# dlilien/ImpDAR

Measured on AMD Instinct MI355X. Metric: migrated traces/sec + achieved HBM GB/s, Kirchhoff 10000x4096 radargram, higher is better.
Workload: dtype f32; 1 GPU; Kirchhoff diffraction-sum migration, 10000 traces x 4096 samples, constant velocity 1.69e8 m/s, dx 1 m, dt 10 ns (BASELINE config 3); kernel=fast, pairs_total=189920188078, pairs_rank0=189920188078, parallelism=output-trace blocks x1, exchange of input-image rows: allgather

## Files before the change

### impdar_amd/csrc/kirch_plan.h

```cpp
#pragma once
#include "common.h"
#include "kirch_route.h"
#include <vector>

#define KF_PAD_ROWS 128

struct impdar_kirch_plan : KirchGeometry, KirchRoute {
    impdar_ctx *ctx = nullptr;
    KirchKnobs knobs;
    int dtype = IMPDAR_F32, snum = 0, tnum = 0, nranks = 1;
    int nearfield = 0;
    int grad_uniform = 0;
    double grad_h = 1.0, vel = 0;
    DevBuf d_XK, d_XW, d_XW2, d_xhmax;
    int xntab = 0;
    bool xtab_ready = false;
    int diag_tables_built = 0;
    bool table_built[2] = {false, false};
    DevBuf d_dist, d_tt, d_zs, d_zs2, d_ga, d_gb, d_gc;
    DevBuf GT[2], DT[2];
    int buf = 0;
    bool migrated_since_prep = false;
    const void *last_out = nullptr;
    int last_out_buf = 0;
    hipEvent_t ev_ready[2] = {nullptr, nullptr};
    hipEvent_t ev_free[2] = {nullptr, nullptr};
    bool free_recorded[2] = {false, false};
    DevBuf d_hmax, d_klo, d_khi;
    DevBuf d_TK[2], d_TW[2], d_TW2[2], d_c1, d_c2, d_fin, d_WIN;
    int nrows = 0, mrow0 = 0;
    int nb = 0, ntab = 0;
    std::vector<int> h_hmax;
    DevBuf d_queue;
    int slots = 0;
    DevBuf d_partial;
    DevBuf d_tilemap;
    std::vector<short> h_tilemap;
    int tm_key[5] = {-1, -1, -1, -1, -1};
    DevBuf d_ga32, d_ga2_32, d_alo2, d_jr;
    std::vector<double> h_dist, h_zs2min;
    std::vector<int2> h_jr;
    int jr_key[2] = {-1, -1};
    int ntie_groups = 0;
    DevBuf d_tie_ti, d_tie_off, d_tie_n;
    DevBuf d_c1d, d_c2d, d_find;
    std::vector<int> h_half;
    int nchunks = 0;
    static constexpr int NSLOT = 64;
    hipEvent_t evs[NSLOT][6] = {};
    bool haves[NSLOT][3] = {};
    int slot = 0;

    ~impdar_kirch_plan()
    {
        for (hipEvent_t e : {ev_ready[0], ev_ready[1], ev_free[0], ev_free[1]})
            if (e) (void)hipEventDestroy(e);
        for (int s = 0; s < NSLOT; ++s)
            for (int i = 0; i < 6; ++i)
                if (evs[s][i]) (void)hipEventDestroy(evs[s][i]);
    }
};

static inline char *img_row0(const impdar_kirch_plan *p, const DevBuf &b)
{
    return reinterpret_cast<char *>(b.p) + (size_t)KF_PAD_ROWS * p->snum * impdar_dtype_size(p->dtype);
}

static int upload(DevBuf &b, const void *src, size_t bytes)
{
    IMPDAR_HIP_CHECK(b.ensure(bytes ? bytes : 8));
    if (bytes) IMPDAR_HIP_CHECK(hipMemcpy(b.p, src, bytes, hipMemcpyHostToDevice));
    return IMPDAR_OK;
}

int kirch_launch_gen(impdar_kirch_plan *p, void *d_out, int xlo, int xhi, hipStream_t st);
```

### impdar_amd/csrc/kirch_route.h

```cpp
#pragma once
#include "../../include/impdar_hip.h"
#include <algorithm>
#include <cmath>
#include <cstdlib>
#include <cstring>
#include <vector>

#if defined(__HIPCC__)
#define KIRCH_HD __host__ __device__
#else
#define KIRCH_HD
#endif

#define KF_THREADS 256
#define KF_W 512

#define KQ_GS 1056
KIRCH_HD constexpr int kq_ring_slots(int xb) { return ((xb + 15 + 7) / 8) * 8; }
KIRCH_HD constexpr int kq_piece_bytes(int xb) { return ((kq_ring_slots(xb) / 8 * KQ_GS + 255) / 256) * 256; }
KIRCH_HD constexpr int kq_piece_bytes_lk(int xb, int lk) { return (((kq_ring_slots(xb) / 8 + lk) * KQ_GS + 255) / 256) * 256; }
static_assert(kq_piece_bytes_lk(40, 0) == 7424 && kq_piece_bytes_lk(40, 1) == 8448 && kq_piece_bytes_lk(24, 0) == 5376, "");
static_assert(kq_ring_slots(24) == 40 && kq_piece_bytes(24) == 5376 && kq_ring_slots(32) == 48 && kq_piece_bytes(32) == 6400 &&
              kq_ring_slots(40) == 56 && kq_piece_bytes(40) == 7424, "");
KIRCH_HD constexpr int kd_ring_slots(int xb) { return ((xb + 7 + 3) / 4) * 4; }
// ... 398 lines not shown
    std::vector<double> load(8, 0.0);
    std::vector<std::pair<double, int>> cost(units);
    for (int c = 0; c < nchunks; ++c) {
        const int hm = h_hmax[c];
        for (int u = 0; u < units; ++u) {
            double w = 0;
            for (int t = u * G; t < std::min((u + 1) * G, nxt); ++t) {
                const int x0 = x00 + t * tile_w;
                const int nlo = std::max(-hm, -(x0 + tile_w - 1)), nhi = std::min(hm, tnum - 1 - x0);
                const int blocks = std::max(0, nhi - nlo + step_block) / step_block;
                w += ((blocks + ring_blocks - 1) / ring_blocks) * ring_blocks + 8;
            }
            cost[u] = {w, u};
        }
        std::sort(cost.begin(), cost.end(), [](const std::pair<double, int> &a, const std::pair<double, int> &b) {
            return a.first > b.first || (a.first == b.first && a.second < b.second);
        });
        int used[8] = {0, 0, 0, 0, 0, 0, 0, 0};
        for (const auto &cu : cost) {
            int best = -1;
            for (int x = 0; x < 8; ++x)
                if (used[x] < cap && (best < 0 || load[x] < load[best])) best = x;
            for (int g = 0; g < G; ++g) {
                const int t = cu.second * G + g;
                map[((size_t)c * tiles_per_xcd + (size_t)used[best] * G + g) * 8 + best] = (short)(t < nxt ? t : -1);
            }
            ++used[best];
            load[best] += cu.first;
        }
    }
    return map;
}

#ifdef KIRCH_ROUTE_PROBE
static inline KirchKnobs kirch_probe_knobs(const int *k)
{
    KirchKnobs K;
    K.xb_set = k[0], K.xb = k[1], K.nh_set = k[2], K.nh = k[3], K.lk_set = k[4], K.lk = k[5], K.parts_set = k[6], K.parts = k[7];
    K.nhd_set = k[8], K.nhd = k[9], K.xbd_set = k[10], K.xbd = k[11], K.impl = k[12], K.exact_impl = k[13], K.tiefix_off = k[14];
    return K;
}

extern "C" int impdar_kirch_route_probe(int dtype, int snum, int tnum, const double *dist_m, const double *tt_sec, double vel, int nearfield,
                                        int mode, int nranks, const double *tmax_override, int caller_tables, const int *knobs,
                                        long long tie_count, long long tie_cap, int *ints, double *dbls)
{
    const KirchGeometry G = kirch_geometry(snum, tnum, dist_m, tt_sec, vel, tmax_override);
    KirchRoute R = kirch_route(G, dtype, snum, tnum, nranks, nearfield, mode, kirch_probe_knobs(knobs), caller_tables != 0);
    if (R.status == IMPDAR_OK && tie_count >= 0) kirch_route_after_ties(R, tie_count, tie_cap);
    const int I[23] = {R.status, R.mode, R.status == IMPDAR_OK ? R.kernel() : -1, R.tnum_pad, R.gen, R.genW, R.quad, R.dquad, R.xb, R.nh, R.lk, R.quadW,
                       R.quadSH, R.walk_parts_log2, R.want_tie_scan, R.xtab_off, R.tie_ambiguous, R.want_tie_groups, G.increasing, G.uni_t,
                       G.uni_t11, G.uni_x, G.dist_sorted};
    const double D[10] = {G.tmax, G.dt, G.dx, G.xnoise, G.sa, G.alpha, G.hest, G.gen_need, R.err_limit, R.err_sa};
    std::copy(I, I + 23, ints);
    std::copy(D, D + 10, dbls);
    return 0;
}

extern "C" int impdar_kirch_tables_probe(int dtype, int snum, int tnum, const double *dist_m, const double *tt_sec, double vel, int nearfield,
                                         int mode, int nranks, const int *knobs, int *sizes, int *h_half, float *c32 ,
                                         double *c64 , float *gen2 , double *gen_chunk ,
                                         int *hmax, int *klo, int *khi, int *win)
{
    const KirchGeometry G = kirch_geometry(snum, tnum, dist_m, tt_sec, vel, nullptr);
    const KirchRoute R = kirch_route(G, dtype, snum, tnum, nranks, nearfield, mode, kirch_probe_knobs(knobs), false);
    if (R.status != IMPDAR_OK || !G.increasing) return -1;
// ... 14 lines not shown
        std::copy(T.zs2min.begin(), T.zs2min.end(), gen_chunk + T.alo2.size());
    }
    if (G.uniform && ((R.mode == IMPDAR_KIRCH_FAST && !R.gen) || R.dquad)) {
        const KirchRingTables T = kirch_ring_tables(G, R, tt_sec, snum, tnum, h);
        const int S[8] = {T.nchunks, T.nb, T.ntab, T.nrows, T.mrow0, T.tkbytes >= ((size_t)1 << 31), (int)T.win.size(), 0};
        std::copy(S, S + 8, sizes);
        if (hmax) std::copy(T.hmax.begin(), T.hmax.end(), hmax);
        if (klo) std::copy(T.klo.begin(), T.klo.end(), klo);
        if (khi) std::copy(T.khi.begin(), T.khi.end(), khi);
        if (win) std::copy(T.win.begin(), T.win.end(), win);
    }
    return 0;
}

extern "C" int impdar_kirch_ties_probe(int *ties, int n, int *g_ti, int *g_off, int *g_n)
{
    std::vector<KirchTie> list(n);
    if (n) memcpy(list.data(), ties, (size_t)n * sizeof(KirchTie));
    const KirchTieGroups T = kirch_group_ties(list);
    std::copy(T.g_ti.begin(), T.g_ti.end(), g_ti);
    std::copy(T.g_off.begin(), T.g_off.end(), g_off);
    std::copy(T.g_n.begin(), T.g_n.end(), g_n);
    return (int)T.g_ti.size();
}

extern "C" int impdar_kirch_tilemap_probe(const int *h_hmax, int nchunks, int tnum, int xlo, int xhi, int tile_w, int align_mask, int ring_blocks,
                                          int step_block, int G, int tiles_per_xcd, short *map)
{
    const std::vector<short> m = kirch_tilemap(std::vector<int>(h_hmax, h_hmax + nchunks), tnum, xlo, xhi, tile_w, align_mask, ring_blocks,
                                               step_block, G, tiles_per_xcd, nchunks);
    std::copy(m.begin(), m.end(), map);
    return (int)m.size();
}
#endif
```

### impdar_amd/csrc/kirchhoff.hip

```cpp
#include "common.h"
#include "kirch_plan.h"
#include <limits>
#include <cmath>
#include <algorithm>
#include <chrono>
#include <memory>
#include <thread>


struct PrepParams {
    const void *data;
    int ld;
    int snum, nloc, jlo;
    void *GT;
    void *DT;
    int grad_uniform;
    int precomputed;
    double grad_h;
    const double *ga, *gb, *gc;
    int clean;
    int i8;
};

template <typename TI, typename TO>
// ... 1570 lines not shown
    if (hipSetDevice(ctx->device) != hipSuccess) {
        impdar_set_error("hipSetDevice(%d) failed: %s", ctx->device, hipGetErrorString(hipGetLastError()));
        return IMPDAR_ERR_HIP;
    }
    const bool own = caller && !caller->standard;
    int rc;
    if ((rc = kirch_alloc_images(p.get())) ||
        (rc = kirch_upload_axes(p.get(), dist_m, tt_sec, ga, gb, gc, own ? caller->zs : nullptr, own ? caller->zs2 : nullptr)) ||
        (p->want_tie_scan && (rc = kirch_tie_scan(p.get()))) ||
        (p->gen && (rc = kirch_upload_gen_tables(p.get(), dist_m, tt_sec))) ||
        (((p->mode == IMPDAR_KIRCH_FAST && !p->gen) || p->dquad) && (rc = kirch_upload_ring_tables(p.get(), tt_sec))) ||
        (rc = kirch_create_events(p.get())))
        return rc;
    *out = p.release();
    return IMPDAR_OK;
}

extern "C" int impdar_kirch_plan_create(impdar_ctx *ctx, int dtype, int snum, int tnum,
                                        const double *dist_m, const double *tt_sec, double vel,
                                        int nearfield, int grad_uniform, double grad_h,
                                        const double *ga, const double *gb, const double *gc,
                                        int mode, int nranks, impdar_kirch_plan **out)
{
    return kirch_plan_create_impl(ctx, dtype, snum, tnum, dist_m, tt_sec, vel, nearfield, grad_uniform, grad_h, ga, gb, gc, mode, nranks,
                                  KirchKnobs::from_env(), nullptr, out);
}

extern "C" void impdar_kirch_plan_destroy(impdar_kirch_plan *p)
{
    if (!p) return;
    (void)hipSetDevice(p->ctx->device);
    (void)hipStreamSynchronize(p->ctx->aux);
    (void)hipStreamSynchronize(p->ctx->stream);
    delete p;
}

extern "C" int impdar_kirch_plan_mode(const impdar_kirch_plan *p) { return p ? p->mode : IMPDAR_ERR_ARG; }
extern "C" double impdar_kirch_plan_xnoise(const impdar_kirch_plan *p) { return p ? p->xnoise : -1.0; }
extern "C" int impdar_kirch_plan_tnum_pad(const impdar_kirch_plan *p) { return p ? p->tnum_pad : IMPDAR_ERR_ARG; }
extern "C" int impdar_kirch_plan_kernel(const impdar_kirch_plan *p) { return p ? p->kernel() : IMPDAR_ERR_ARG; }

static int prep_image(impdar_kirch_plan *p, const void *d_data, int ld, int jlo, int nloc, int precomputed, int b, hipStream_t st)
{
    PrepParams P;
    P.data = d_data;
    P.ld = ld;
    P.snum = p->snum;
    P.nloc = nloc;
    P.jlo = jlo;
    P.GT = img_row0(p, p->GT[b]);
    P.DT = p->nearfield ? img_row0(p, p->DT[b]) : nullptr;
    P.grad_uniform = p->grad_uniform;
    P.precomputed = precomputed;
    P.grad_h = p->grad_h;
    P.ga = p->d_ga.as<double>();
    P.gb = p->d_gb.as<double>();
    P.gc = p->d_gc.as<double>();
    P.clean = (p->mode == IMPDAR_KIRCH_FAST) ? 1 : (p->dquad ? 2 : 0);
    P.i8 = (p->quad || p->dquad) ? 1 : 0;
    dim3 grid((nloc + 63) / 64, (p->snum + 63) / 64);
    if (p->dtype == IMPDAR_F32 && P.i8)
        hipLaunchKernelGGL((kirch_prep_direct_kernel<float, 8>), dim3((nloc + 255) / 256, p->snum), dim3(256), 0, st, P);
    else if (p->dquad)
        hipLaunchKernelGGL((kirch_prep_direct_kernel<double, 4>), dim3((nloc + 255) / 256, p->snum), dim3(256), 0, st, P);
    else if (p->dtype == IMPDAR_F32)
        hipLaunchKernelGGL((kirch_prep_kernel<float, float>), grid, dim3(256), 0, st, P);
// ... 63 lines not shown
        p->haves[p->slot][0] = p->haves[p->slot][1] = p->haves[p->slot][2] = false;
    }
    const int b = p->buf;
    if (p->free_recorded[b] && !more) IMPDAR_HIP_CHECK(hipStreamWaitEvent(st, p->ev_free[b], 0));
    if (p->ctx->produced) IMPDAR_HIP_CHECK(hipStreamWaitEvent(st, p->ctx->ev_produced, 0));
    if (p->last_out && d_data == p->last_out && p->free_recorded[p->last_out_buf])
        IMPDAR_HIP_CHECK(hipStreamWaitEvent(st, p->ev_free[p->last_out_buf], 0));
    hipEvent_t *ev = p->evs[p->slot];
    if (!p->haves[p->slot][0]) IMPDAR_HIP_CHECK(hipEventRecord(ev[0], st));
    int rc;
    if (nloc > 0 && (rc = prep_image(p, d_data, ld, jlo, nloc, precomputed, b, st))) return rc;
    if ((p->mode == IMPDAR_KIRCH_FAST && p->quad) || p->dquad)
        rc = prep_table_ring(p, b, st);
    else
        rc = (p->mode == IMPDAR_KIRCH_FAST && !p->gen) ? prep_table_tab(p, b, st) : IMPDAR_OK;
    if (rc) return rc;
    IMPDAR_HIP_CHECK(hipEventRecord(ev[1], st));
    IMPDAR_HIP_CHECK(hipEventRecord(p->ev_ready[b], st));
    p->haves[p->slot][0] = true;
    return IMPDAR_OK;
}

extern "C" int impdar_kirch_prep(impdar_kirch_plan *p, const void *d_data, int ld, int jlo, int nloc)
{
    return kirch_prep_impl(p, d_data, ld, jlo, nloc, 0);
}

int impdar_kirch_prep_precomputed(impdar_kirch_plan *p, const void *d_grad, int ld, int jlo, int nloc)
{
    return kirch_prep_impl(p, d_grad, ld, jlo, nloc, 1);
}

static int build_tilemap(impdar_kirch_plan *p, FastParams &P, int tile_w, int align_mask, int ring_blocks, int step_block,
                         hipStream_t st)
{
    P.tilemap = nullptr;
    const int key[5] = {P.xlo, P.xhi, tile_w, P.G, P.tiles_per_xcd};
    const size_t n = (size_t)P.nchunks * P.tiles_per_xcd * 8;
    if (memcmp(key, p->tm_key, sizeof(key)) != 0 || p->h_tilemap.size() != n) {
        std::vector<short> map = kirch_tilemap(p->h_hmax, p->tnum, P.xlo, P.xhi, tile_w, align_mask, ring_blocks, step_block, P.G,
                                               P.tiles_per_xcd, P.nchunks);
        if (map.empty()) return IMPDAR_OK;
        p->h_tilemap.swap(map);
        memcpy(p->tm_key, key, sizeof(key));
        IMPDAR_HIP_CHECK(p->d_tilemap.ensure(n * sizeof(short)));
        IMPDAR_HIP_CHECK(hipMemcpyAsync(p->d_tilemap.p, p->h_tilemap.data(), n * sizeof(short), hipMemcpyHostToDevice, st));
    }
    P.tilemap = p->d_tilemap.as<short>();
    return IMPDAR_OK;
}

#ifndef KQ_DEFAULT_RESERVE
#define KQ_DEFAULT_RESERVE 32
#endif
static int kirch_reserved_slots(const impdar_kirch_plan *p)
{
    const char *re = getenv("IMPDAR_KIRCH_RESERVE");
    const int r = re ? atoi(re) : (p->nranks > 1 ? KQ_DEFAULT_RESERVE : 0);
    return std::min(std::max(r, 0), 256);
}

template <typename T>
static void kirch_launch_combine(const FastParams &P, hipStream_t st)
{
    const size_t nout = (size_t)P.snum * P.ldo;
    const dim3 cg((unsigned)((nout + 255) / 256));
    if (P.parts_log2 == 2)
        hipLaunchKernelGGL((kirch_combine_kernel<T, 4>), cg, dim3(256), 0, st, (const T *)P.partial, (T *)P.out, nout);
    else
        hipLaunchKernelGGL((kirch_combine_kernel<T, 2>), cg, dim3(256), 0, st, (const T *)P.partial, (T *)P.out, nout);
}

template <int XB_, int OCC, int SH, int NH_ = 1, int LK = 0>
struct RingF32 {
    static constexpr int XB = XB_, NH = NH_;
    static constexpr int align_mask = 7, step_block = 8, ring_blocks = (kq_ring_slots(XB) + 8 * LK) / 8, piece_bytes = kq_piece_bytes_lk(XB, LK);
    static auto near_kernel() { return kirch_quad_kernel<XB, true, 1, SH, 1, 0>; }
    static auto far_kernel() { return kirch_quad_kernel<XB, false, OCC, SH, NH, LK>; }
};
template <int XB_, int SH, int NH_ = 1>
struct RingF64 {
    static constexpr int XB = XB_, NH = NH_;
    static constexpr int align_mask = 3, step_block = 4, ring_blocks = kd_ring_slots(XB) / 4, piece_bytes = kd_piece_bytes(XB);
    static auto near_kernel() { return kirch_dquad_kernel<XB, true, 1, SH, 1>; }
    static auto far_kernel() { return kirch_dquad_kernel<XB, false, (NH > 1 ? 4 : 2), SH, NH>; }
};

template <typename K>
static int launch_ring(impdar_kirch_plan *p, const FastParams &P0, hipStream_t st)
{
    constexpr int XB = K::XB, NH = K::NH;
    FastParams P = P0;
    const int ntiles = (P.xhi - (P.xlo & ~K::align_mask) + XB * NH - 1) / (XB * NH);
    P.nxt = ntiles;
    P.G = ntiles >= 256 ? 4 : 1;
    const int per = 8 * P.G;
    const int nxt_pad = ((ntiles + per - 1) / per) * per;
    P.tiles_per_xcd = nxt_pad / 8;
    const int nblk = P.nchunks * nxt_pad;
    const int W = p->quadW;
    {
        const int trc = build_tilemap(p, P, XB * NH, K::align_mask, K::ring_blocks, K::step_block, st);
        if (trc) return trc;
    }
    const size_t shmem = (size_t)(W / 32) * K::piece_bytes * (p->nearfield ? 2 : 1) + 16;
    if (p->nearfield) {
        auto k = K::near_kernel();
        IMPDAR_HIP_CHECK(hipFuncSetAttribute((const void *)k, hipFuncAttributeMaxDynamicSharedMemorySize, (int)shmem));
        hipLaunchKernelGGL(k, dim3(nblk), dim3(KF_THREADS), shmem, st, P, W);
        IMPDAR_HIP_CHECK(hipGetLastError());
        return IMPDAR_OK;
    }
    auto k = K::far_kernel();
    IMPDAR_HIP_CHECK(hipFuncSetAttribute((const void *)k, hipFuncAttributeMaxDynamicSharedMemorySize, (int)shmem));
    int grid = nblk;
    if (P.tilemap) {
        if (p->slots <= 0) {
            int per_cu = 0, ncu = 0;
            if (hipOccupancyMaxActiveBlocksPerMultiprocessor(&per_cu, (const void *)k, KF_THREADS * NH, shmem) == hipSuccess &&
                hipDeviceGetAttribute(&ncu, hipDeviceAttributeMultiprocessorCount, p->ctx->device) == hipSuccess &&
                per_cu > 0 && ncu > 0)
                p->slots = per_cu * ncu;
            else
                (void)hipGetLastError();
        }
        const int pl2 = NH == 1 ? p->walk_parts_log2 : 0;
        const size_t nout = (size_t)P.snum * P.ldo, esz = impdar_dtype_size(p->dtype);
        const bool pieces = pl2 > 0 && p->slots > 0 && p->d_partial.ensure((nout << pl2) * esz) == hipSuccess;
        if (p->slots > 0 && (p->slots < nblk || pieces) && p->d_queue.ensure(8 * 64) == hipSuccess) {
            IMPDAR_HIP_CHECK(hipMemsetAsync(p->d_queue.p, 0, 8 * 64, st));
            P.queue = p->d_queue.as<int>();
            if (pieces) {
                P.parts_log2 = pl2;
                P.partial = p->d_partial.p;
                P.part_stride = nout;
                IMPDAR_HIP_CHECK(hipMemsetAsync(p->d_partial.p, 0, (nout << pl2) * esz, st));
            }
            grid = (int)std::min<long long>(std::max(p->slots - kirch_reserved_slots(p), 1), (long long)nblk << P.parts_log2);
        }
    }
    hipLaunchKernelGGL(k, dim3(grid), dim3(KF_THREADS * NH), shmem, st, P, W);
    if (P.parts_log2 && p->dtype == IMPDAR_F32) kirch_launch_combine<float>(P, st);
    if (P.parts_log2 && p->dtype != IMPDAR_F32) kirch_launch_combine<double>(P, st);
    IMPDAR_HIP_CHECK(hipGetLastError());
    return IMPDAR_OK;
}

template <int XB, int S, int OCC>
static int launch_tab(impdar_kirch_plan *p, const FastParams &P0, int nx, hipStream_t st)
{
    constexpr int R = XB + 2 * S;
    FastParams P = P0;
    const int ntiles = (nx + XB - 1) / XB;
    P.nxt = ntiles;
    P.G = 4;
    const int per = 8 * P.G;
    const int nxt_pad = ((ntiles + per - 1) / per) * per;
    P.tiles_per_xcd = nxt_pad / 8;
    const int nblk = P.nchunks * nxt_pad;
    const size_t shmem = (size_t)R * KF_W * 4 * (p->nearfield ? 2 : 1);
    if (p->nearfield) {
        auto k = kirch_tab_kernel<XB, S, true, 1>;
        IMPDAR_HIP_CHECK(hipFuncSetAttribute((const void *)k, hipFuncAttributeMaxDynamicSharedMemorySize, (int)shmem));
        hipLaunchKernelGGL(k, dim3(nblk), dim3(KF_THREADS), shmem, st, P);
    } else {
        auto k = kirch_tab_kernel<XB, S, false, OCC>;
        IMPDAR_HIP_CHECK(hipFuncSetAttribute((const void *)k, hipFuncAttributeMaxDynamicSharedMemorySize, (int)shmem));
        hipLaunchKernelGGL(k, dim3(nblk), dim3(KF_THREADS), shmem, st, P);
    }
    IMPDAR_HIP_CHECK(hipGetLastError());
    return IMPDAR_OK;
}

static int migrate_ring(impdar_kirch_plan *p, void *d_out, int xlo, int xhi, hipStream_t st)
{
    const int b = p->buf, nx = xhi - xlo;
    FastParams P;
    P.GT = reinterpret_cast<const float *>(img_row0(p, p->GT[b]));
    P.DT = p->nearfield ? reinterpret_cast<const float *>(img_row0(p, p->DT[b])) : nullptr;
    P.out = reinterpret_cast<float *>(d_out);
    P.ldo = nx;
    P.snum = p->snum;
    P.tnum = p->tnum;
    P.xlo = xlo;
    P.xhi = xhi;
    P.hmax = p->d_hmax.as<int>();
    P.klo = p->d_klo.as<int>();
    P.khi = p->d_khi.as<int>();
    P.nb = p->nb;
    P.zero_row = p->tnum_pad;
    P.nchunks = p->nchunks;
    P.TK = p->d_TK[b].as<unsigned short>();
    P.TW = p->d_TW[b].as<float>();
    P.TW2 = p->d_TW2[b].as<float>();
    P.ntab = p->ntab;
    P.c1 = p->d_c1.as<float>();
    P.c2 = p->d_c2.as<float>();
    P.fin = p->d_fin.as<float>();
    P.c1d = p->d_c1d.as<double>();
    P.c2d = p->d_c2d.as<double>();
    P.find = p->d_find.as<double>();
    P.TKB = p->d_TK[b].p;
    P.WIN = p->d_WIN.as<int2>();
    P.nrows = p->nrows;
    P.mrow0 = p->mrow0;
    P.tilemap = nullptr;
    P.queue = nullptr;
    P.parts_log2 = 0;
    P.partial = nullptr;
    P.part_stride = 0;
    if (p->dquad && p->nh == 2 && p->quadSH == 4)
        return p->xb == 20 ? launch_ring<RingF64<20, 4, 2>>(p, P, st) : launch_ring<RingF64<16, 4, 2>>(p, P, st);
    if (p->dquad)
        return p->quadSH == 0 ? (p->xb == 20 ? launch_ring<RingF64<20, 0>>(p, P, st) : launch_ring<RingF64<16, 0>>(p, P, st))
                              : (p->xb == 20 ? launch_ring<RingF64<20, 4>>(p, P, st) : launch_ring<RingF64<16, 4>>(p, P, st));
    if (p->quad && p->quadSH == 0)
        return p->xb == 40 ? launch_ring<RingF32<40, 2, 0>>(p, P, st)
               : p->xb == 32 ? launch_ring<RingF32<32, 2, 0>>(p, P, st)
                             : launch_ring<RingF32<24, 3, 0>>(p, P, st);
    if (p->quad && p->nh == 2 && p->xb == 32)
        return launch_ring<RingF32<32, 4, 4, 2, 0>>(p, P, st);
    if (p->quad && p->nh == 2 && p->xb == 40)
        return p->lk ? launch_ring<RingF32<40, 2, 4, 2, 1>>(p, P, st) : launch_ring<RingF32<40, 2, 4, 2, 0>>(p, P, st);
    if (p->quad && p->nh == 3 && p->xb == 40)
        return p->lk ? launch_ring<RingF32<40, 3, 4, 3, 1>>(p, P, st) : launch_ring<RingF32<40, 3, 4, 3, 0>>(p, P, st);
    if (p->quad)
        return p->xb == 40 ? launch_ring<RingF32<40, 2, 4>>(p, P, st)
               : p->xb == 32 ? launch_ring<RingF32<32, 2, 4>>(p, P, st)
                             : launch_ring<RingF32<24, 2, 4>>(p, P, st);
    return launch_tab<16, 4, 4>(p, P, nx, st);
}

static int build_exact_tables(impdar_kirch_plan *p, hipStream_t st)
{
    const int nch = (p->snum + 255) / 256;
    int hg = 0;
    std::vector<int> hm(nch, 0);
    for (int k = 0; k < p->snum; ++k) {
        hm[k / 256] = std::max(hm[k / 256], p->h_half[k] + 1);
        hg = std::max(hg, p->h_half[k] + 1);
    }
    hg = std::min(hg, p->tnum) + 1;
    const size_t ent = (size_t)hg * p->snum;
    if (p->d_XK.ensure(ent * 4) != hipSuccess || p->d_XW.ensure(ent * 8) != hipSuccess ||
        (p->nearfield && p->d_XW2.ensure(ent * 8) != hipSuccess) || p->d_xhmax.ensure((size_t)nch * 4) != hipSuccess) {
        impdar_set_error("hipMalloc of the %zu-entry exact pick/weight table failed", ent);
        return IMPDAR_ERR_HIP;
    }
    IMPDAR_HIP_CHECK(hipMemcpyAsync(p->d_xhmax.p, hm.data(), (size_t)nch * 4, hipMemcpyHostToDevice, st));
    IMPDAR_HIP_CHECK(hipStreamSynchronize(st));
    TableXParams T;
    T.XK = p->d_XK.as<int>();
    T.XW = p->d_XW.as<double>();
    T.XW2 = p->d_XW2.as<double>();
    kirch_fill_axes(T, p);
    T.dx = p->dx;
    T.ntab = hg;
    T.near = p->nearfield;
    hipLaunchKernelGGL(kirch_tablex_kernel, dim3(nch, hg), dim3(256), 0, st, T);
    IMPDAR_HIP_CHECK(hipGetLastError());
    p->xntab = hg;
    p->xtab_ready = true;
// ... 50 lines not shown
        if (p->nearfield)
            hipLaunchKernelGGL((kirch_exact_kernel<double, true>), grid, dim3(256), 0, st, P);
        else
            hipLaunchKernelGGL((kirch_exact_kernel<double, false>), grid, dim3(256), 0, st, P);
    }
    IMPDAR_HIP_CHECK(hipGetLastError());
    return IMPDAR_OK;
}

static int migrate_tiefix(impdar_kirch_plan *p, int kern, void *d_out, int xlo, int xhi, hipStream_t st)
{
    TieFixParams F;
    kirch_fill_io(F, p, d_out, xlo, xhi);
    kirch_fill_axes(F, p);
    F.grp = kern == IMPDAR_KERNEL_QUAD ? 8 : (kern == IMPDAR_KERNEL_DQUAD ? 4 : 0);
    F.near = p->nearfield;
    F.dist = p->d_dist.as<double>();
    F.dx = p->dx;
    F.g_ti = p->d_tie_ti.as<int>();
    F.g_off = p->d_tie_off.as<int>();
    F.g_n = p->d_tie_n.as<int>();
    const bool xtab = kern == IMPDAR_KERNEL_EXACT_TAB;
    F.hmax = xtab ? p->d_xhmax.as<int>() : p->d_hmax.as<int>();
    F.nmax = xtab ? p->xntab : p->ntab - 1;
    const dim3 grid((xhi - xlo + 255) / 256, p->ntie_groups);
    if (p->dtype == IMPDAR_F32)
        hipLaunchKernelGGL(kirch_tiefix_kernel<float>, grid, dim3(256), 0, st, F);
    else
        hipLaunchKernelGGL(kirch_tiefix_kernel<double>, grid, dim3(256), 0, st, F);
    IMPDAR_HIP_CHECK(hipGetLastError());
    return IMPDAR_OK;
}

extern "C" int impdar_kirch_migrate(impdar_kirch_plan *p, void *d_out, int xlo, int xhi)
{
    IMPDAR_ARG_CHECK(p && d_out, "null plan/output");
    IMPDAR_ARG_CHECK(0 <= xlo && xlo <= xhi && xhi <= p->tnum, "bad output trace range [%d,%d) for tnum %d", xlo,
                     xhi, p->tnum);
    IMPDAR_HIP_CHECK(hipSetDevice(p->ctx->device));
    hipStream_t st = p->ctx->stream;
    hipEvent_t *ev = p->evs[p->slot];
    const int b = p->buf;
    IMPDAR_HIP_CHECK(hipStreamWaitEvent(st, p->ev_ready[b], 0));
    if (!p->haves[p->slot][2]) IMPDAR_HIP_CHECK(hipEventRecord(ev[4], st));
    const int kern = p->kernel();
    if (xhi > xlo) {
        const int rc = kern == IMPDAR_KERNEL_GEN          ? kirch_launch_gen(p, d_out, xlo, xhi, st)
                       : kern == IMPDAR_KERNEL_EXACT_TAB  ? migrate_exact_tab(p, d_out, xlo, xhi, st)
                       : kern == IMPDAR_KERNEL_EXACT_PAIR ? migrate_exact_pair(p, d_out, xlo, xhi, st)
                                                          : migrate_ring(p, d_out, xlo, xhi, st);
        if (rc) return rc;
        if (p->ntie_groups > 0 && kern != IMPDAR_KERNEL_EXACT_PAIR) {
            const int frc = migrate_tiefix(p, kern, d_out, xlo, xhi, st);
            if (frc) return frc;
        }
    }
    IMPDAR_HIP_CHECK(hipEventRecord(ev[5], st));
    IMPDAR_HIP_CHECK(hipEventRecord(p->ev_free[b], st));
    p->free_recorded[b] = true;
    p->last_out = d_out;
    p->last_out_buf = b;
    p->migrated_since_prep = true;
    p->haves[p->slot][2] = true;
    return IMPDAR_OK;
}

int impdar_allgather_rows(impdar_ctx *ctx, void *image, size_t bytes_per_rank, hipStream_t stream);

extern "C" int impdar_kirch_allgather(impdar_kirch_plan *p)
{
    IMPDAR_ARG_CHECK(p, "null plan");
    IMPDAR_ARG_CHECK(p->nranks == p->ctx->nranks || getenv("IMPDAR_COMM_EMULATE"),
                     "plan was built for %d ranks but the communicator has %d", p->nranks, p->ctx->nranks);
    IMPDAR_HIP_CHECK(hipSetDevice(p->ctx->device));
    hipStream_t st = p->ctx->aux;
    hipEvent_t *ev = p->evs[p->slot];
    const int b = p->buf;
    IMPDAR_HIP_CHECK(hipEventRecord(ev[2], st));
    if (p->nranks > 1 || p->ctx->comm) {
        const size_t per = (size_t)(p->tnum_pad / p->nranks) * p->snum * impdar_dtype_size(p->dtype);
        int rc = impdar_allgather_rows(p->ctx, img_row0(p, p->GT[b]), per, st);
        if (rc) return rc;
        if (p->nearfield && (rc = impdar_allgather_rows(p->ctx, img_row0(p, p->DT[b]), per, st))) return rc;
    }
    IMPDAR_HIP_CHECK(hipEventRecord(ev[3], st));
    IMPDAR_HIP_CHECK(hipEventRecord(p->ev_ready[b], st));
    p->haves[p->slot][1] = true;
    return IMPDAR_OK;
}

int impdar_exchange_ranges(impdar_ctx *ctx, void *image, int nsend, const int *speer, const size_t *soff,
                           const size_t *slen, int nrecv, const int *rpeer, const size_t *roff, const size_t *rlen,
                           hipStream_t stream);
// ... 141 lines not shown
                     c.nearfield == nearfield && c.grad_uniform == grad_uniform && c.grad_h == grad_h && c.mode == mode &&
                     dist_m && tt_sec && same_vec(c.dist, dist_m, (size_t)tnum) && same_vec(c.tt, tt_sec, (size_t)snum) &&
                     same_vec(c.ga, ga, (size_t)snum) && same_vec(c.gb, gb, (size_t)snum) &&
                     same_vec(c.gc, gc, (size_t)snum) && c.knobs == knobs;
    int rc;
    if (!hit) {
        c.drop();
        if ((rc = kirch_plan_create_impl(ctx, dtype, snum, tnum, dist_m, tt_sec, vel, nearfield, grad_uniform, grad_h,
                                         ga, gb, gc, mode, 1, knobs, nullptr, &c.plan))) {
            c.plan = nullptr;
            return rc;
        }
        c.owner = ctx;
        c.dtype = dtype, c.snum = snum, c.tnum = tnum, c.nearfield = nearfield, c.grad_uniform = grad_uniform, c.mode = mode;
        c.vel = vel, c.grad_h = grad_h;
        c.dist.assign(dist_m, dist_m + tnum);
        c.tt.assign(tt_sec, tt_sec + snum);
        auto take = [&](std::vector<double> &v, const double *p) {
            if (p) v.assign(p, p + snum);
            else v.clear();
        };
        take(c.ga, ga);
        take(c.gb, gb);
        take(c.gc, gc);
        c.knobs = knobs;
    }
    impdar_kirch_plan *p = c.plan;
    const size_t esz = impdar_dtype_size(dtype);
    const size_t bytes = (size_t)snum * tnum * esz;
    auto done = [&](int code) {
        if (code != IMPDAR_OK) {
            (void)hipStreamSynchronize(ctx->aux);
            (void)hipStreamSynchronize(ctx->stream);
        }
        if (code != IMPDAR_OK || !keep) c.drop();
        return code;
    };
    if (c.din.ensure(bytes) != hipSuccess || c.dout.ensure(bytes) != hipSuccess) {
        impdar_set_error("hipMalloc of %zu bytes failed", bytes);
        return done(IMPDAR_ERR_HIP);
    }
    const auto t0b = now();
    const char *se = getenv("IMPDAR_KIRCH_ONESHOT_SPLIT");
    const int kern = impdar_kirch_plan_kernel(p);
    const bool split = !(se && atoi(se) == 0) && tnum >= 4096 && bytes >= ((size_t)64 << 20) &&
                       (kern == IMPDAR_KERNEL_QUAD || kern == IMPDAR_KERNEL_DQUAD);
    impdar_ctx_pinned_prefetch(ctx, std::min(bytes, IMPDAR_STAGE_RING_BYTES));
    int nlaunch = 1;
    if (split) {
        const int halo = p->ntab + 16;
        auto r8 = [](long long x) { return (int)(x / 8 * 8); };
        std::vector<int> cut;
        const bool two = se && atoi(se) == 2;
#ifndef KOS_PCT
#define KOS_PCT {10, 40, 70}
#endif
        const std::vector<int> pct = KOS_PCT;
        if (!two && (long long)tnum * pct[pct.size() > 1 ? 1 : 0] / 100 + halo < (long long)tnum * 9 / 10) {
            cut = {0};
            for (int q : pct) cut.push_back(r8((long long)tnum * q / 100));
            cut.push_back(tnum);
        } else {
            cut = {0, r8((long long)tnum * 5 / 8), tnum};
        }
        const int nblk = (int)cut.size() - 1;
        nlaunch = nblk;
        for (int i = 0; i < nblk; ++i)
            if (!c.ev_blk[i] && hipEventCreateWithFlags(&c.ev_blk[i], hipEventDisableTiming) != hipSuccess) {
                c.ev_blk[i] = nullptr;
                impdar_set_error("hipEventCreate failed");
                return done(IMPDAR_ERR_HIP);
            }
        char *dout = reinterpret_cast<char *>(c.dout.p);
        int have = 0;
        for (int i = 0; i < nblk; ++i) {
            const int need = two ? tnum : (int)std::min<long long>(tnum, ((long long)cut[i + 1] + halo + 7) / 8 * 8);
            if (need > have) {
                if (hipMemcpy2DAsync(reinterpret_cast<char *>(c.din.p) + (size_t)have * esz, (size_t)tnum * esz,
                                     reinterpret_cast<const char *>(data) + (size_t)have * esz, (size_t)tnum * esz,
                                     (size_t)(need - have) * esz, (size_t)snum, hipMemcpyHostToDevice, ctx->aux) != hipSuccess) {
                    impdar_set_error("H2D copy failed");
                    return done(IMPDAR_ERR_HIP);
                }
                if ((rc = kirch_prep_impl(p, reinterpret_cast<const char *>(c.din.p) + (size_t)have * esz, tnum, have,
                                          need - have, 0, have > 0)))
                    return done(rc);
                have = need;
            }
            if ((rc = impdar_kirch_migrate(p, dout + (size_t)snum * cut[i] * esz, cut[i], cut[i + 1]))) return done(rc);
            if (hipEventRecord(c.ev_blk[i], ctx->stream) != hipSuccess) return done(IMPDAR_ERR_HIP);
        }
        {
            std::vector<size_t> col0(nblk), width(nblk);
            std::vector<const void *> src(nblk);
            for (int i = 0; i < nblk; ++i) {
                col0[i] = (size_t)cut[i];
                width[i] = (size_t)(cut[i + 1] - cut[i]);
                src[i] = dout + (size_t)snum * cut[i] * esz;
            }
            if ((rc = impdar_download_blocks_f64(ctx, out, (size_t)tnum, (size_t)snum, dtype, nblk, col0.data(), width.data(),
                                                 src.data(), c.ev_blk, ctx->aux)))
                return done(rc);
        }
    } else {
        if (hipMemcpyAsync(c.din.p, data, bytes, hipMemcpyHostToDevice, ctx->stream) != hipSuccess ||
            hipStreamSynchronize(ctx->stream) != hipSuccess) {
            impdar_set_error("H2D copy failed");
            return done(IMPDAR_ERR_HIP);
        }
        if ((rc = impdar_kirch_prep(p, c.din.p, tnum, 0, tnum))) return done(rc);
        if ((rc = impdar_kirch_migrate(p, c.dout.p, 0, tnum))) return done(rc);
        if ((rc = impdar_dev_download_f64(ctx, out, c.dout.p, dtype, (size_t)snum * tnum))) return done(rc);
    }
    float kms = -1.f;
    {
        float a = 0.f, b = 0.f, c2 = 0.f;
        if (impdar_kirch_last_ms(p, &a, &b, &c2) == IMPDAR_OK) kms = c2;
        (void)hipGetLastError();
    }
    static const char *kernel_names[] = {"kirch_exact_kernel", "kirch_exact_tab_kernel", "kirch_dquad_kernel", "kirch_quad_kernel",
                                         "kirch_tab_kernel", "kirch_gen_kernel"};
    ctx->m_entry = "impdar_kirchhoff";
    ctx->m_kernel = (kern >= 0 && kern < 6) ? kernel_names[kern] : "";
    ctx->m_kernel_ms = kms;
    ctx->timed = false;
    const auto t2 = now();
    const bool offset_weighted = kern == IMPDAR_KERNEL_DQUAD || kern == IMPDAR_KERNEL_EXACT_TAB;
    snprintf(ctx->m_extra, sizeof ctx->m_extra,
             "\"plan\": \"%s\", \"launches\": %d, \"plan_ms\": %.3f, \"call_ms\": %.3f, \"xnoise\": %.3g, \"parity_bar\": %.3g",
             hit ? "cached" : "new", nlaunch, ms(t0, t0b), ms(t0, t2), p->xnoise,
             dtype == IMPDAR_F32 && p->mode == IMPDAR_KIRCH_FAST ? 1e-4 : (offset_weighted ? std::max(1e-12, 0.1 * p->xnoise) : 1e-12));
    rc = done(IMPDAR_OK);
    return rc;
}

int impdar_kirch_prep_precomputed(impdar_kirch_plan *p, const void *d_grad, int ld, int jlo, int nloc);

namespace {
struct KirchHook {
    impdar_ctx *ctx = nullptr;
    impdar_kirch_plan *plan = nullptr;
    DevBuf din, dout;
    int snum = 0, tnum = 0;
    double vel = 0, tmax = 0;
    bool standard = false;
    std::vector<double> dist, tt, zs, zs2;
    KirchKnobs knobs;
    void drop()
    {
        if (plan) impdar_kirch_plan_destroy(plan);
        plan = nullptr;
        din.release();
        dout.release();
    }
};
std::mutex g_hook_mu;
KirchHook g_hook;
}

void impdar_kirch_trim()
{
    if (!t_k1_busy) {
        std::unique_lock<std::mutex> lk(g_k1_mu, std::try_to_lock);
// ... 73 lines not shown
```

Before: 1.319 million traces/s.

## Pipeline one-shot Kirchhoff blocks across two streams with per-block tilemaps and queues

The one-shot Kirchhoff path now splits the migration into more blocks (default cut points 10/30/50/70/85/95 percent instead of 10/40/70). Consecutive blocks alternate between the main stream and a second stream. Each block gets its own tilemap cache and work-queue counters, so blocks on the two streams can run at once and overlap with the staged H2D copies and prep. The goal is to hide the tail of each block's kernel and the upload latency. The costs are extra launches, shared bandwidth between the two concurrent kernels, and more tilemap builds per call.

```diff
diff --git a/impdar_amd/csrc/kirch_plan.h b/impdar_amd/csrc/kirch_plan.h
--- a/impdar_amd/csrc/kirch_plan.h
+++ b/impdar_amd/csrc/kirch_plan.h
@@ -37,6 +37,17 @@
     DevBuf d_tilemap;
     std::vector<short> h_tilemap;
     int tm_key[5] = {-1, -1, -1, -1, -1};
+    struct BlockSlot {
+        DevBuf d_tilemap;
+        std::vector<short> h_tilemap;
+        int tm_key[5] = {-1, -1, -1, -1, -1};
+        int *queue = nullptr;
+    };
+    BlockSlot blk[KOS_NBLK];
+    DevBuf d_blkqueue;
+    hipStream_t stream2 = nullptr;
+    hipEvent_t ev_fork = nullptr;
+    int diag_slot_maps_built = 0;
     DevBuf d_ga32, d_ga2_32, d_alo2, d_jr;
     std::vector<double> h_dist, h_zs2min;
     std::vector<int2> h_jr;
@@ -58,6 +69,8 @@
         for (int s = 0; s < NSLOT; ++s)
             for (int i = 0; i < 6; ++i)
                 if (evs[s][i]) (void)hipEventDestroy(evs[s][i]);
+        if (ev_fork) (void)hipEventDestroy(ev_fork);
+        if (stream2) (void)hipStreamDestroy(stream2);
     }
 };
 
diff --git a/impdar_amd/csrc/kirch_route.h b/impdar_amd/csrc/kirch_route.h
--- a/impdar_amd/csrc/kirch_route.h
+++ b/impdar_amd/csrc/kirch_route.h
@@ -454,6 +454,82 @@
     return map;
 }
 
+#define KOS_NBLK 8
+#ifndef KOS_PCT
+#define KOS_PCT {10, 30, 50, 70, 85, 95}
+#endif
+struct KirchOneShotPlan {
+    bool pipelined = false;
+    int nblk = 1;
+    int cut[KOS_NBLK + 1] = {};
+    int need[KOS_NBLK] = {};
+    int stream[KOS_NBLK] = {};
+};
+
+static inline int kirch_oneshot_cuts(int tnum, int halo, const int *pct, int npct, bool two, int *cut, int *need)
+{
+    auto r8 = [](long long x) { return (int)(x / 8 * 8); };
+    bool ok = pct && npct >= 1 && npct <= KOS_NBLK - 1;
+    for (int i = 0; ok && i < npct; ++i) ok = pct[i] >= 1 && pct[i] <= 99 && (i == 0 || pct[i] > pct[i - 1]);
+    const int dflt[] = KOS_PCT;
+    if (!ok) pct = dflt, npct = (int)(sizeof(dflt) / sizeof(dflt[0]));
+    int n = 0;
+    cut[0] = 0;
+    auto add = [&](int c) {
+        if (c > cut[n] && c < tnum) cut[++n] = c;
+    };
+    if (!two && (long long)tnum * pct[npct > 1 ? 1 : 0] / 100 + halo < (long long)tnum * 9 / 10)
+        for (int i = 0; i < npct; ++i) add(r8((long long)tnum * pct[i] / 100));
+    else
+        add(r8((long long)tnum * 5 / 8));
+    cut[++n] = tnum;
+    for (int i = 0; i < n; ++i)
+        need[i] = two ? tnum : (int)std::min<long long>(tnum, ((long long)cut[i + 1] + halo + 7) / 8 * 8);
+    return n;
+}
+
+struct KirchOneShotKnob {
+    int split = -1;
+    int npct = 0;
+    int pct[KOS_NBLK] = {};
+};
+static inline KirchOneShotKnob kirch_oneshot_knob(const char *s)
+{
+    KirchOneShotKnob K;
+    if (!s) return K;
+    K.split = atoi(s);
+    const char *q = strchr(s, ':');
+    if (!q) return K;
+    for (++q;;) {
+        char *end = nullptr;
+        const long v = strtol(q, &end, 10);
+        const bool bad = end == q || (*end && *end != ',') || K.npct >= KOS_NBLK - 1;
+        if (bad) {
+            K.npct = 1;
+            K.pct[0] = -1;
+            return K;
+        }
+        K.pct[K.npct++] = (int)std::min<long>(std::max<long>(v, -1), 1000);
+        if (!*end) return K;
+        q = end + 1;
+    }
+}
+
+static inline KirchOneShotPlan kirch_oneshot_plan(int tnum, long long bytes, int halo, int kernel, int split, const int *pct, int npct)
+{
+    KirchOneShotPlan O;
+    O.cut[1] = O.need[0] = tnum;
+    const bool ring = kernel == IMPDAR_KERNEL_QUAD || kernel == IMPDAR_KERNEL_DQUAD;
+    if (split == 0 || !ring || tnum < 1 || halo < 0) return O;
+    if (split != 3 && !(tnum >= 4096 && bytes >= ((long long)64 << 20))) return O;
+    KirchOneShotPlan S;
+    S.nblk = kirch_oneshot_cuts(tnum, halo, pct, npct, split == 2, S.cut, S.need);
+    if (S.nblk < 2) return O;
+    S.pipelined = true;
+    for (int i = 0; i < S.nblk; ++i) S.stream[i] = i & 1;
+    return S;
+}
+
 #ifdef KIRCH_ROUTE_PROBE
 static inline KirchKnobs kirch_probe_knobs(const int *k)
 {
@@ -534,4 +610,23 @@
     std::copy(m.begin(), m.end(), map);
     return (int)m.size();
 }
-#endif
+
+extern "C" int impdar_kirch_oneshot_probe(int tnum, long long bytes, int halo, int kernel, int split, const int *pct, int npct, int *pipelined,
+                                          int *cut, int *need, int *stream)
+{
+    const KirchOneShotPlan O = kirch_oneshot_plan(tnum, bytes, halo, kernel, split, npct ? pct : nullptr, npct);
+    *pipelined = O.pipelined;
+    std::copy(O.cut, O.cut + KOS_NBLK + 1, cut);
+    std::copy(O.need, O.need + KOS_NBLK, need);
+    std::copy(O.stream, O.stream + KOS_NBLK, stream);
+    return O.nblk;
+}
+
+extern "C" int impdar_kirch_oneshot_knob_probe(const char *s, int *split, int *pct)
+{
+    const KirchOneShotKnob K = kirch_oneshot_knob(s);
+    *split = K.split;
+    std::copy(K.pct, K.pct + KOS_NBLK, pct);
+    return K.npct;
+}
+#endif
diff --git a/impdar_amd/csrc/kirchhoff.hip b/impdar_amd/csrc/kirchhoff.hip
--- a/impdar_amd/csrc/kirchhoff.hip
+++ b/impdar_amd/csrc/kirchhoff.hip
@@ -1626,6 +1626,7 @@
     (void)hipSetDevice(p->ctx->device);
     (void)hipStreamSynchronize(p->ctx->aux);
     (void)hipStreamSynchronize(p->ctx->stream);
+    if (p->stream2) (void)hipStreamSynchronize(p->stream2);
     delete p;
 }
 
@@ -1755,21 +1756,25 @@
 }
 
 static int build_tilemap(impdar_kirch_plan *p, FastParams &P, int tile_w, int align_mask, int ring_blocks, int step_block,
-                         hipStream_t st)
+                         hipStream_t st, impdar_kirch_plan::BlockSlot *ls)
 {
     P.tilemap = nullptr;
     const int key[5] = {P.xlo, P.xhi, tile_w, P.G, P.tiles_per_xcd};
     const size_t n = (size_t)P.nchunks * P.tiles_per_xcd * 8;
-    if (memcmp(key, p->tm_key, sizeof(key)) != 0 || p->h_tilemap.size() != n) {
+    int *have_key = ls ? ls->tm_key : p->tm_key;
+    std::vector<short> &h_map = ls ? ls->h_tilemap : p->h_tilemap;
+    DevBuf &d_map = ls ? ls->d_tilemap : p->d_tilemap;
+    if (memcmp(key, have_key, sizeof(key)) != 0 || h_map.size() != n) {
         std::vector<short> map = kirch_tilemap(p->h_hmax, p->tnum, P.xlo, P.xhi, tile_w, align_mask, ring_blocks, step_block, P.G,
                                                P.tiles_per_xcd, P.nchunks);
         if (map.empty()) return IMPDAR_OK;
-        p->h_tilemap.swap(map);
-        memcpy(p->tm_key, key, sizeof(key));
-        IMPDAR_HIP_CHECK(p->d_tilemap.ensure(n * sizeof(short)));
-        IMPDAR_HIP_CHECK(hipMemcpyAsync(p->d_tilemap.p, p->h_tilemap.data(), n * sizeof(short), hipMemcpyHostToDevice, st));
-    }
-    P.tilemap = p->d_tilemap.as<short>();
+        h_map.swap(map);
+        memcpy(have_key, key, sizeof(key));
+        IMPDAR_HIP_CHECK(d_map.ensure(n * sizeof(short)));
+        IMPDAR_HIP_CHECK(hipMemcpyAsync(d_map.p, h_map.data(), n * sizeof(short), hipMemcpyHostToDevice, st));
+        if (ls) ++p->diag_slot_maps_built;
+    }
+    P.tilemap = d_map.as<short>();
     return IMPDAR_OK;
 }
 
@@ -1810,7 +1815,7 @@
 };
 
 template <typename K>
-static int launch_ring(impdar_kirch_plan *p, const FastParams &P0, hipStream_t st)
+static int launch_ring(impdar_kirch_plan *p, const FastParams &P0, hipStream_t st, impdar_kirch_plan::BlockSlot *ls)
 {
     constexpr int XB = K::XB, NH = K::NH;
     FastParams P = P0;
@@ -1823,7 +1828,7 @@
     const int nblk = P.nchunks * nxt_pad;
     const int W = p->quadW;
     {
-        const int trc = build_tilemap(p, P, XB * NH, K::align_mask, K::ring_blocks, K::step_block, st);
+        const int trc = build_tilemap(p, P, XB * NH, K::align_mask, K::ring_blocks, K::step_block, st, ls);
         if (trc) return trc;
     }
     const size_t shmem = (size_t)(W / 32) * K::piece_bytes * (p->nearfield ? 2 : 1) + 16;
@@ -1850,9 +1855,13 @@
         const int pl2 = NH == 1 ? p->walk_parts_log2 : 0;
         const size_t nout = (size_t)P.snum * P.ldo, esz = impdar_dtype_size(p->dtype);
         const bool pieces = pl2 > 0 && p->slots > 0 && p->d_partial.ensure((nout << pl2) * esz) == hipSuccess;
-        if (p->slots > 0 && (p->slots < nblk || pieces) && p->d_queue.ensure(8 * 64) == hipSuccess) {
-            IMPDAR_HIP_CHECK(hipMemsetAsync(p->d_queue.p, 0, 8 * 64, st));
-            P.queue = p->d_queue.as<int>();
+        if (p->slots > 0 && (p->slots < nblk || pieces) && ((ls && ls->queue) || p->d_queue.ensure(8 * 64) == hipSuccess)) {
+            if (ls && ls->queue) {
+                P.queue = ls->queue;
+            } else {
+                IMPDAR_HIP_CHECK(hipMemsetAsync(p->d_queue.p, 0, 8 * 64, st));
+                P.queue = p->d_queue.as<int>();
+            }
             if (pieces) {
                 P.parts_log2 = pl2;
                 P.partial = p->d_partial.p;
@@ -1895,7 +1904,7 @@
     return IMPDAR_OK;
 }
 
-static int migrate_ring(impdar_kirch_plan *p, void *d_out, int xlo, int xhi, hipStream_t st)
+static int migrate_ring(impdar_kirch_plan *p, void *d_out, int xlo, int xhi, hipStream_t st, impdar_kirch_plan::BlockSlot *ls)
 {
     const int b = p->buf, nx = xhi - xlo;
     FastParams P;
@@ -1933,24 +1942,24 @@
     P.partial = nullptr;
     P.part_stride = 0;
     if (p->dquad && p->nh == 2 && p->quadSH == 4)
-        return p->xb == 20 ? launch_ring<RingF64<20, 4, 2>>(p, P, st) : launch_ring<RingF64<16, 4, 2>>(p, P, st);
+        return p->xb == 20 ? launch_ring<RingF64<20, 4, 2>>(p, P, st, ls) : launch_ring<RingF64<16, 4, 2>>(p, P, st, ls);
     if (p->dquad)
-        return p->quadSH == 0 ? (p->xb == 20 ? launch_ring<RingF64<20, 0>>(p, P, st) : launch_ring<RingF64<16, 0>>(p, P, st))
-                              : (p->xb == 20 ? launch_ring<RingF64<20, 4>>(p, P, st) : launch_ring<RingF64<16, 4>>(p, P, st));
+        return p->quadSH == 0 ? (p->xb == 20 ? launch_ring<RingF64<20, 0>>(p, P, st, ls) : launch_ring<RingF64<16, 0>>(p, P, st, ls))
+                              : (p->xb == 20 ? launch_ring<RingF64<20, 4>>(p, P, st, ls) : launch_ring<RingF64<16, 4>>(p, P, st, ls));
     if (p->quad && p->quadSH == 0)
-        return p->xb == 40 ? launch_ring<RingF32<40, 2, 0>>(p, P, st)
-               : p->xb == 32 ? launch_ring<RingF32<32, 2, 0>>(p, P, st)
-                             : launch_ring<RingF32<24, 3, 0>>(p, P, st);
+        return p->xb == 40 ? launch_ring<RingF32<40, 2, 0>>(p, P, st, ls)
+               : p->xb == 32 ? launch_ring<RingF32<32, 2, 0>>(p, P, st, ls)
+                             : launch_ring<RingF32<24, 3, 0>>(p, P, st, ls);
     if (p->quad && p->nh == 2 && p->xb == 32)
-        return launch_ring<RingF32<32, 4, 4, 2, 0>>(p, P, st);
+        return launch_ring<RingF32<32, 4, 4, 2, 0>>(p, P, st, ls);
     if (p->quad && p->nh == 2 && p->xb == 40)
-        return p->lk ? launch_ring<RingF32<40, 2, 4, 2, 1>>(p, P, st) : launch_ring<RingF32<40, 2, 4, 2, 0>>(p, P, st);
+        return p->lk ? launch_ring<RingF32<40, 2, 4, 2, 1>>(p, P, st, ls) : launch_ring<RingF32<40, 2, 4, 2, 0>>(p, P, st, ls);
     if (p->quad && p->nh == 3 && p->xb == 40)
-        return p->lk ? launch_ring<RingF32<40, 3, 4, 3, 1>>(p, P, st) : launch_ring<RingF32<40, 3, 4, 3, 0>>(p, P, st);
+        return p->lk ? launch_ring<RingF32<40, 3, 4, 3, 1>>(p, P, st, ls) : launch_ring<RingF32<40, 3, 4, 3, 0>>(p, P, st, ls);
     if (p->quad)
-        return p->xb == 40 ? launch_ring<RingF32<40, 2, 4>>(p, P, st)
-               : p->xb == 32 ? launch_ring<RingF32<32, 2, 4>>(p, P, st)
-                             : launch_ring<RingF32<24, 2, 4>>(p, P, st);
+        return p->xb == 40 ? launch_ring<RingF32<40, 2, 4>>(p, P, st, ls)
+               : p->xb == 32 ? launch_ring<RingF32<32, 2, 4>>(p, P, st, ls)
+                             : launch_ring<RingF32<24, 2, 4>>(p, P, st, ls);
     return launch_tab<16, 4, 4>(p, P, nx, st);
 }
 
@@ -2067,6 +2076,19 @@
     return IMPDAR_OK;
 }
 
+static int kirch_migrate_launch(impdar_kirch_plan *p, void *d_out, int xlo, int xhi, hipStream_t st, impdar_kirch_plan::BlockSlot *ls)
+{
+    const int kern = p->kernel();
+    if (xhi <= xlo) return IMPDAR_OK;
+    const int rc = kern == IMPDAR_KERNEL_GEN          ? kirch_launch_gen(p, d_out, xlo, xhi, st)
+                   : kern == IMPDAR_KERNEL_EXACT_TAB  ? migrate_exact_tab(p, d_out, xlo, xhi, st)
+                   : kern == IMPDAR_KERNEL_EXACT_PAIR ? migrate_exact_pair(p, d_out, xlo, xhi, st)
+                                                      : migrate_ring(p, d_out, xlo, xhi, st, ls);
+    if (rc) return rc;
+    if (p->ntie_groups > 0 && kern != IMPDAR_KERNEL_EXACT_PAIR) return migrate_tiefix(p, kern, d_out, xlo, xhi, st);
+    return IMPDAR_OK;
+}
+
 extern "C" int impdar_kirch_migrate(impdar_kirch_plan *p, void *d_out, int xlo, int xhi)
 {
     IMPDAR_ARG_CHECK(p && d_out, "null plan/output");
@@ -2078,22 +2100,61 @@
     const int b = p->buf;
     IMPDAR_HIP_CHECK(hipStreamWaitEvent(st, p->ev_ready[b], 0));
     if (!p->haves[p->slot][2]) IMPDAR_HIP_CHECK(hipEventRecord(ev[4], st));
-    const int kern = p->kernel();
-    if (xhi > xlo) {
-        const int rc = kern == IMPDAR_KERNEL_GEN          ? kirch_launch_gen(p, d_out, xlo, xhi, st)
-                       : kern == IMPDAR_KERNEL_EXACT_TAB  ? migrate_exact_tab(p, d_out, xlo, xhi, st)
-                       : kern == IMPDAR_KERNEL_EXACT_PAIR ? migrate_exact_pair(p, d_out, xlo, xhi, st)
-                                                          : migrate_ring(p, d_out, xlo, xhi, st);
+    {
+        const int rc = kirch_migrate_launch(p, d_out, xlo, xhi, st, nullptr);
         if (rc) return rc;
-        if (p->ntie_groups > 0 && kern != IMPDAR_KERNEL_EXACT_PAIR) {
-            const int frc = migrate_tiefix(p, kern, d_out, xlo, xhi, st);
-            if (frc) return frc;
-        }
     }
     IMPDAR_HIP_CHECK(hipEventRecord(ev[5], st));
     IMPDAR_HIP_CHECK(hipEventRecord(p->ev_free[b], st));
     p->free_recorded[b] = true;
     p->last_out = d_out;
+    p->last_out_buf = b;
+    p->migrated_since_prep = true;
+    p->haves[p->slot][2] = true;
+    return IMPDAR_OK;
+}
+
+static int kirch_blocks_begin(impdar_kirch_plan *p, int nblk)
+{
+    IMPDAR_ARG_CHECK(p && nblk >= 1 && nblk <= KOS_NBLK, "a one-shot call has 1 to %d blocks (got %d)", KOS_NBLK, nblk);
+    IMPDAR_HIP_CHECK(hipSetDevice(p->ctx->device));
+    hipStream_t st = p->ctx->stream;
+    if (!p->stream2) {
+        int prio = 0;
+        IMPDAR_HIP_CHECK(hipStreamGetPriority(st, &prio));
+        IMPDAR_HIP_CHECK(hipStreamCreateWithPriority(&p->stream2, hipStreamNonBlocking, prio));
+    }
+    if (!p->ev_fork) IMPDAR_HIP_CHECK(hipEventCreateWithFlags(&p->ev_fork, hipEventDisableTiming));
+    IMPDAR_HIP_CHECK(p->d_blkqueue.ensure((size_t)KOS_NBLK * 8 * 64));
+    for (int i = 0; i < KOS_NBLK; ++i) p->blk[i].queue = p->d_blkqueue.as<int>() + (size_t)i * 8 * 16;
+    IMPDAR_HIP_CHECK(hipStreamWaitEvent(st, p->ev_ready[p->buf], 0));
+    IMPDAR_HIP_CHECK(hipMemsetAsync(p->d_blkqueue.p, 0, (size_t)nblk * 8 * 64, st));
+    if (!p->haves[p->slot][2]) IMPDAR_HIP_CHECK(hipEventRecord(p->evs[p->slot][4], st));
+    IMPDAR_HIP_CHECK(hipEventRecord(p->ev_fork, st));
+    IMPDAR_HIP_CHECK(hipStreamWaitEvent(p->stream2, p->ev_fork, 0));
+    return IMPDAR_OK;
+}
+
+static int kirch_block_launch(impdar_kirch_plan *p, int i, int which, void *d_out, int xlo, int xhi, hipEvent_t summed)
+{
+    IMPDAR_ARG_CHECK(i >= 0 && i < KOS_NBLK && 0 <= xlo && xlo <= xhi && xhi <= p->tnum, "bad block %d [%d,%d) for tnum %d", i, xlo, xhi, p->tnum);
+    hipStream_t st = which ? p->stream2 : p->ctx->stream;
+    IMPDAR_HIP_CHECK(hipStreamWaitEvent(st, p->ev_ready[p->buf], 0));
+    const int rc = kirch_migrate_launch(p, d_out, xlo, xhi, st, &p->blk[i]);
+    if (rc) return rc;
+    IMPDAR_HIP_CHECK(hipEventRecord(summed, st));
+    return IMPDAR_OK;
+}
+
+static int kirch_blocks_end(impdar_kirch_plan *p, void *d_out_last, hipEvent_t last2)
+{
+    hipStream_t st = p->ctx->stream;
+    const int b = p->buf;
+    if (last2) IMPDAR_HIP_CHECK(hipStreamWaitEvent(st, last2, 0));
+    IMPDAR_HIP_CHECK(hipEventRecord(p->evs[p->slot][5], st));
+    IMPDAR_HIP_CHECK(hipEventRecord(p->ev_free[b], st));
+    p->free_recorded[b] = true;
+    p->last_out = d_out_last;
     p->last_out_buf = b;
     p->migrated_since_prep = true;
     p->haves[p->slot][2] = true;
@@ -2301,6 +2362,7 @@
         if (code != IMPDAR_OK) {
             (void)hipStreamSynchronize(ctx->aux);
             (void)hipStreamSynchronize(ctx->stream);
+            if (c.plan && c.plan->stream2) (void)hipStreamSynchronize(c.plan->stream2);
         }
         if (code != IMPDAR_OK || !keep) c.drop();
         return code;
@@ -2310,29 +2372,17 @@
         return done(IMPDAR_ERR_HIP);
     }
     const auto t0b = now();
-    const char *se = getenv("IMPDAR_KIRCH_ONESHOT_SPLIT");
+    const KirchOneShotKnob knob = kirch_oneshot_knob(getenv("IMPDAR_KIRCH_ONESHOT_SPLIT"));
     const int kern = impdar_kirch_plan_kernel(p);
-    const bool split = !(se && atoi(se) == 0) && tnum >= 4096 && bytes >= ((size_t)64 << 20) &&
-                       (kern == IMPDAR_KERNEL_QUAD || kern == IMPDAR_KERNEL_DQUAD);
+    const int halo = p->ntab + 16;
+    const KirchOneShotPlan O = kirch_oneshot_plan(tnum, (long long)bytes, halo, kern, knob.split, knob.npct ? knob.pct : nullptr, knob.npct);
+    const bool split = O.pipelined;
     impdar_ctx_pinned_prefetch(ctx, std::min(bytes, IMPDAR_STAGE_RING_BYTES));
     int nlaunch = 1;
+    const int maps0 = p->diag_slot_maps_built;
     if (split) {
-        const int halo = p->ntab + 16;
-        auto r8 = [](long long x) { return (int)(x / 8 * 8); };
-        std::vector<int> cut;
-        const bool two = se && atoi(se) == 2;
-#ifndef KOS_PCT
-#define KOS_PCT {10, 40, 70}
-#endif
-        const std::vector<int> pct = KOS_PCT;
-        if (!two && (long long)tnum * pct[pct.size() > 1 ? 1 : 0] / 100 + halo < (long long)tnum * 9 / 10) {
-            cut = {0};
-            for (int q : pct) cut.push_back(r8((long long)tnum * q / 100));
-            cut.push_back(tnum);
-        } else {
-            cut = {0, r8((long long)tnum * 5 / 8), tnum};
-        }
-        const int nblk = (int)cut.size() - 1;
+        const int *cut = O.cut;
+        const int nblk = O.nblk;
         nlaunch = nblk;
         for (int i = 0; i < nblk; ++i)
             if (!c.ev_blk[i] && hipEventCreateWithFlags(&c.ev_blk[i], hipEventDisableTiming) != hipSuccess) {
@@ -2342,8 +2392,9 @@
             }
         char *dout = reinterpret_cast<char *>(c.dout.p);
         int have = 0;
+        hipEvent_t last2 = nullptr;
         for (int i = 0; i < nblk; ++i) {
-            const int need = two ? tnum : (int)std::min<long long>(tnum, ((long long)cut[i + 1] + halo + 7) / 8 * 8);
+            const int need = O.need[i];
             if (need > have) {
                 if (hipMemcpy2DAsync(reinterpret_cast<char *>(c.din.p) + (size_t)have * esz, (size_t)tnum * esz,
                                      reinterpret_cast<const char *>(data) + (size_t)have * esz, (size_t)tnum * esz,
@@ -2356,9 +2407,13 @@
                     return done(rc);
                 have = need;
             }
-            if ((rc = impdar_kirch_migrate(p, dout + (size_t)snum * cut[i] * esz, cut[i], cut[i + 1]))) return done(rc);
-            if (hipEventRecord(c.ev_blk[i], ctx->stream) != hipSuccess) return done(IMPDAR_ERR_HIP);
-        }
+            if (i == 0 && (rc = kirch_blocks_begin(p, nblk))) return done(rc);
+            const int which = p->walk_parts_log2 ? 0 : O.stream[i];
+            if ((rc = kirch_block_launch(p, i, which, dout + (size_t)snum * cut[i] * esz, cut[i], cut[i + 1], c.ev_blk[i])))
+                return done(rc);
+            if (which) last2 = c.ev_blk[i];
+        }
+        if ((rc = kirch_blocks_end(p, dout + (size_t)snum * cut[nblk - 1] * esz, last2))) return done(rc);
         {
             std::vector<size_t> col0(nblk), width(nblk);
             std::vector<const void *> src(nblk);
@@ -2396,8 +2451,8 @@
     const auto t2 = now();
     const bool offset_weighted = kern == IMPDAR_KERNEL_DQUAD || kern == IMPDAR_KERNEL_EXACT_TAB;
     snprintf(ctx->m_extra, sizeof ctx->m_extra,
-             "\"plan\": \"%s\", \"launches\": %d, \"plan_ms\": %.3f, \"call_ms\": %.3f, \"xnoise\": %.3g, \"parity_bar\": %.3g",
-             hit ? "cached" : "new", nlaunch, ms(t0, t0b), ms(t0, t2), p->xnoise,
+             "\"plan\": \"%s\", \"launches\": %d, \"slot_maps_built\": %d, \"plan_ms\": %.3f, \"call_ms\": %.3f, \"xnoise\": %.3g, \"parity_bar\": %.3g",
+             hit ? "cached" : "new", nlaunch, p->diag_slot_maps_built - maps0, ms(t0, t0b), ms(t0, t2), p->xnoise,
              dtype == IMPDAR_F32 && p->mode == IMPDAR_KIRCH_FAST ? 1e-4 : (offset_weighted ? std::max(1e-12, 0.1 * p->xnoise) : 1e-12));
     rc = done(IMPDAR_OK);
     return rc;
```

Result: no change. 1.318 million traces/s, median of 3 (-0.1%).
